# tanmayrainanda/ishara

Hardware: AMD Instinct MI355X
Metric: landmark-frames/sec training (B=256,T=384,d=256) (higher is better)
Workload: dtype bf16; 1 GPU; configs[1]: get_model(dim=256, 2 squeeze + 2 conformer blocks, kernel_sizes=[11,5,3]) CTC train step (fwd+CTC+bwd+RAdam/Lookahead, dropout on); batch_per_gpu=256, global_batch=256, frames=384, features=224, params=7577784, parallelism=dp1, ranks_seen=1

## Files before the change

### include/ishara_hip.h

```cpp
#ifndef ISHARA_HIP_H
#define ISHARA_HIP_H
#include <stdint.h>
#ifdef __cplusplus
extern "C" {
#endif

typedef struct ishara_model ishara_model;
typedef void* ishara_stream;

enum { ISHARA_F32 = 0, ISHARA_BF16 = 1, ISHARA_F16 = 2 };
enum { ISHARA_FAMILY_KERAS_HYBRID = 0, ISHARA_FAMILY_TORCH_CONFORMER = 1, ISHARA_FAMILY_TORCH_SQUEEZEFORMER = 2 };

typedef struct ishara_config {
    int32_t dim;
    int32_t num_conv_squeeze_blocks;
    int32_t num_conv_conform_blocks;
    int32_t num_kernel_sizes;
    int32_t kernel_sizes[8];
    int32_t num_conv_per_block;
    float   dropout_rate;
    int32_t num_heads;
    int32_t expansion_factor;
    int32_t transformer_kernel_size;
    int32_t frames;
// ... 69 lines not shown
                         int32_t* dist, int32_t* tlen, ishara_stream s);

int64_t ishara_ctc_beam_workspace_bytes(int32_t B, int32_t T, int32_t C, int32_t beam_width);
int ishara_ctc_beam_decode(const float* logits, int32_t B, int32_t T, int32_t C, int32_t blank, int32_t beam_width, int32_t nbest,
                           const float* lm, float alpha, float beta, void* workspace,
                           int32_t* out_idx, int32_t* out_len, float* out_score, ishara_stream s);

int64_t ishara_ctc_align_workspace_bytes(int32_t B, int32_t T, int32_t L);
int ishara_ctc_align(const float* logits, const int64_t* labels, int32_t B, int32_t T, int32_t C, int32_t L, int32_t blank,
                     void* ws, int32_t* frame_pos, int32_t* start, int32_t* end, float* conf, float* score, ishara_stream s);

typedef struct ishara_clip_aug {
    int64_t offset;
    int32_t n;
    int32_t L1;
    int32_t shift;
    int32_t L2;
    int32_t mirror;
    int32_t t0[3];
    int32_t t1[3];
    int32_t fingers[3];
} ishara_clip_aug;
enum { ISHARA_LAYOUT_FLAT = 0, ISHARA_LAYOUT_HANDS_LIPS_XY = 1 };
int ishara_clip_batch(const float* raw, const ishara_clip_aug* clips, int32_t B, int32_t T, int32_t layout,
                      float* x, ishara_stream s);
int64_t ishara_ctc_workspace_bytes(int32_t B, int32_t T, int32_t L);
int ishara_ctc_loss(const float* logits, const int64_t* labels, int32_t B, int32_t T, int32_t C,
                    int32_t L, int32_t blank, float* nll, float* dlogits, float grad_scale,
                    void* ws, ishara_stream s);
int ishara_dropout_mask(uint32_t seed, uint32_t site, int32_t rows, int32_t cols, float rate,
                        float* out, ishara_stream s);

int ishara_debug_set_as_flags(int32_t flags);
int ishara_debug_set_nt_big(int32_t on);
int ishara_debug_force_regstage(int32_t on);
int32_t ishara_debug_module_count(ishara_model* m);
int ishara_debug_module_info(ishara_model* m, int32_t i, const char** name, int32_t* in_cols, int32_t* out_cols, int32_t* first_site, int32_t* n_sites);
int ishara_debug_module_forward(ishara_model* m, int32_t i, const float* x, int32_t B, float* y, int32_t training, uint32_t seed, ishara_stream s);
int ishara_debug_module_backward(ishara_model* m, int32_t i, const float* dy, int32_t B, float* dx, ishara_stream s);
int ishara_debug_head_loss_backward(ishara_model* m, const float* logits, const int64_t* labels, int32_t B, float* loss, float* nll,
                                    float loss_scale, float* dx, ishara_stream s);

int64_t ishara_op_scratch_bytes(int32_t M, int32_t K, int32_t N);
int ishara_op_dense_fwd(int32_t dt, const void* x, const float* W, const float* bias, void* y,
                        int32_t M, int32_t K, int32_t N, int32_t act, void* scratch, ishara_stream s);
int ishara_op_dense_fwd_ex(int32_t dt, const void* x, const float* W, const float* bias, const void* resid, void* y,
                           int32_t M, int32_t K, int32_t N, int32_t act, void* scratch, ishara_stream s);
int ishara_op_dense_bwd(int32_t dt, const void* x, const float* W, const void* dy, void* dx,
                        float* dW, float* db, int32_t M, int32_t K, int32_t N, void* scratch, ishara_stream s);
int64_t ishara_op_qkv_scratch_bytes(int32_t B, int32_t T, int32_t H, int32_t dh);
int ishara_op_qkv_fwd(int32_t dt, const void* x, const float* gamma, const float* beta, float eps, const float* W, const float* bias,
                      void* q, void* k, void* vt, int32_t B, int32_t T, int32_t H, int32_t dh, int32_t head_major, void* scratch, ishara_stream s);
int ishara_op_classifier_fwd(int32_t dt, const void* x, const float* W, const float* bias, float* logits, int32_t M, int32_t K, int32_t C,
                             int32_t route, void* scratch, ishara_stream s);
int ishara_op_ctc_loss(const float* logits, const int64_t* labels, int32_t B, int32_t T, int32_t C, int32_t L, int32_t blank,
                       float* nll, float* dlogits, float grad_scale, void* ws, void* dlb, ishara_stream s);
int ishara_op_log_softmax_fwd(const float* x, float* y, int32_t M, int32_t C, int32_t ld, ishara_stream s);
int ishara_op_log_softmax_bwd(const float* dy, const float* y, float* dx, int32_t M, int32_t C, int32_t ld, ishara_stream s);
int ishara_op_layernorm_fwd(int32_t dt, const void* x, const float* gamma, const float* beta, float eps,
                            void* y, float* mean, float* rstd, int32_t M, int32_t C, ishara_stream s);
int ishara_op_layernorm_bwd(int32_t dt, const void* dy, const void* x, const float* mean, const float* rstd,
                            const float* gamma, void* dx, float* dgamma, float* dbeta, int32_t M, int32_t C,
                            ishara_stream s);
int ishara_op_dwconv_fwd(int32_t dt, int32_t inop, const void* x, const float* w, const float* bias, void* y,
                         float* ssum, float* ssq, int32_t B, int32_t T, int32_t C, int32_t k, int32_t padl,
                         ishara_stream s);
// ... 44 lines not shown
```

### ishara_amd/_lib.py

```python
from __future__ import annotations

import ctypes as C
import os

_HERE = os.path.dirname(os.path.abspath(__file__))
LIB_PATH = os.path.join(_HERE, "libishara_hip.so")

F32, BF16, F16 = 0, 1, 2
FAMILY_KERAS_HYBRID, FAMILY_TORCH_CONFORMER, FAMILY_TORCH_SQUEEZEFORMER = 0, 1, 2


class IsharaError(RuntimeError):
    pass


class Config(C.Structure):
    _fields_ = [
        ("dim", C.c_int32), ("num_conv_squeeze_blocks", C.c_int32), ("num_conv_conform_blocks", C.c_int32),
        ("num_kernel_sizes", C.c_int32), ("kernel_sizes", C.c_int32 * 8), ("num_conv_per_block", C.c_int32),
        ("dropout_rate", C.c_float), ("num_heads", C.c_int32), ("expansion_factor", C.c_int32),
        ("transformer_kernel_size", C.c_int32), ("frames", C.c_int32), ("features", C.c_int32),
        ("num_classes", C.c_int32), ("top_dim", C.c_int32), ("squeeze_expansion", C.c_int32),
        ("conformer_expansion", C.c_int32), ("head_dropout", C.c_float), ("conformer_attn_dropout", C.c_float),
        ("dtype", C.c_int32), ("max_batch", C.c_int32), ("max_label_len", C.c_int32), ("attn_impl", C.c_int32),
# ... 31 lines not shown
    "ishara_grad_bucket": (C.c_int, [_P, _I32, C.POINTER(C.c_int64), C.POINTER(C.c_int64)]),
    "ishara_grad_buckets_enable": (C.c_int, [_P]),
    "ishara_grad_bucket_wait": (C.c_int, [_P, _I32, _P]),
    "ishara_bind": (C.c_int, [_P, _P, _P, _P, _P, _P, _P, _I64]),
    "ishara_sync_weights": (C.c_int, [_P, _P]),
    "ishara_forward": (C.c_int, [_P, _P, _I32, _P, _I32, _U32, _P]),
    "ishara_encoder_forward": (C.c_int, [_P, _P, _I32, _P, _I32, _U32, _P]),
    "ishara_encoder_backward": (C.c_int, [_P, _P, _I32, _P, _P]),
    "ishara_encoder_output_frames": (_I32, [_P]),
    "ishara_loss_backward": (C.c_int, [_P, _P, _P, _I32, _P, _P, _F, _P]),
    "ishara_optimizer_step": (C.c_int, [_P, _F, _F, _P]),
    "ishara_optimizer_iterations": (_I32, [_P]),
    "ishara_optimizer_set_iterations": (C.c_int, [_P, _I32]),
    "ishara_grad_stats_workspace_bytes": (_I64, [_I64]),
    "ishara_gradient_stats": (C.c_int, [_P, _P, _I64, _F, _F, _P, _P, _P]),
    "ishara_gradient_accumulate": (C.c_int, [_P, _P, _P, _I64, _I32, _P]),
    "ishara_optimizer_step_ex": (C.c_int, [_P, _F, _F, _P, _P, _I32, _P]),
    "ishara_profile_enable": (C.c_int, [_P, _I32]),
    "ishara_profile_report": (C.c_int, [_P, C.c_char_p, _I32]),
    "ishara_greedy_decode": (C.c_int, [_P, _I32, _I32, _I32, _I32, _P, _P, _P]),
    "ishara_preprocess": (C.c_int, [_P, _P, _I32, _P, _P, _P, _I32, _P]),
    "ishara_preprocess_batch": (C.c_int, [_P, _I64, _P, _I32, _I32, _P, _P, _P, _I32, _P]),
    "ishara_edit_distance": (C.c_int, [_P, _P, _I32, _I32, _P, _I32, _P, _P, _P]),
    "ishara_ctc_beam_workspace_bytes": (_I64, [_I32, _I32, _I32, _I32]),
    "ishara_ctc_beam_decode": (C.c_int, [_P, _I32, _I32, _I32, _I32, _I32, _I32, _P, _F, _F, _P, _P, _P, _P, _P]),
    "ishara_ctc_align_workspace_bytes": (_I64, [_I32, _I32, _I32]),
    "ishara_ctc_align": (C.c_int, [_P, _P, _I32, _I32, _I32, _I32, _I32, _P, _P, _P, _P, _P, _P, _P]),
    "ishara_clip_batch": (C.c_int, [_P, _P, _I32, _I32, _I32, _P, _P]),
    "ishara_ctc_workspace_bytes": (_I64, [_I32, _I32, _I32]),
    "ishara_ctc_loss": (C.c_int, [_P, _P, _I32, _I32, _I32, _I32, _I32, _P, _P, _F, _P, _P]),
    "ishara_op_ctc_loss": (C.c_int, [_P, _P, _I32, _I32, _I32, _I32, _I32, _P, _P, _F, _P, _P, _P]),
    "ishara_dropout_mask": (C.c_int, [_U32, _U32, _I32, _I32, _F, _P, _P]),
    "ishara_debug_set_as_flags": (C.c_int, [_I32]),
    "ishara_debug_set_nt_big": (C.c_int, [_I32]),
    "ishara_debug_force_regstage": (C.c_int, [_I32]),
    "ishara_debug_module_count": (_I32, [_P]),
    "ishara_debug_module_info": (C.c_int, [_P, _I32, C.POINTER(C.c_char_p), C.POINTER(_I32), C.POINTER(_I32), C.POINTER(_I32), C.POINTER(_I32)]),
    "ishara_debug_module_forward": (C.c_int, [_P, _I32, _P, _I32, _P, _I32, _U32, _P]),
    "ishara_debug_module_backward": (C.c_int, [_P, _I32, _P, _I32, _P, _P]),
    "ishara_debug_head_loss_backward": (C.c_int, [_P, _P, _P, _I32, _P, _P, _F, _P, _P]),
    "ishara_op_scratch_bytes": (_I64, [_I32, _I32, _I32]),
    "ishara_op_dense_fwd": (C.c_int, [_I32, _P, _P, _P, _P, _I32, _I32, _I32, _I32, _P, _P]),
    "ishara_op_dense_fwd_ex": (C.c_int, [_I32, _P, _P, _P, _P, _P, _I32, _I32, _I32, _I32, _P, _P]),
    "ishara_op_dense_bwd": (C.c_int, [_I32, _P, _P, _P, _P, _P, _P, _I32, _I32, _I32, _P, _P]),
    "ishara_op_qkv_scratch_bytes": (_I64, [_I32, _I32, _I32, _I32]),
    "ishara_op_qkv_fwd": (C.c_int, [_I32, _P, _P, _P, _F, _P, _P, _P, _P, _P, _I32, _I32, _I32, _I32, _I32, _P, _P]),
    "ishara_op_classifier_fwd": (C.c_int, [_I32, _P, _P, _P, _P, _I32, _I32, _I32, _I32, _P, _P]),
    "ishara_op_log_softmax_fwd": (C.c_int, [_P, _P, _I32, _I32, _I32, _P]),
    "ishara_op_log_softmax_bwd": (C.c_int, [_P, _P, _P, _I32, _I32, _I32, _P]),
    "ishara_op_layernorm_fwd": (C.c_int, [_I32, _P, _P, _P, _F, _P, _P, _P, _I32, _I32, _P]),
    "ishara_op_layernorm_bwd": (C.c_int, [_I32, _P, _P, _P, _P, _P, _P, _P, _P, _I32, _I32, _P]),
    "ishara_op_dwconv_fwd": (C.c_int, [_I32, _I32, _P, _P, _P, _P, _P, _P, _I32, _I32, _I32, _I32, _I32, _P]),
    "ishara_op_dwconv_scratch_bytes": (_I64, [_I32, _I32]),
    "ishara_op_dwconv_fwd_scratch_bytes": (_I64, [_I32, _I32, _I32]),
    "ishara_op_dwconv_fwd_ex": (C.c_int, [_I32, _I32, _P, _P, _P, _P, _P, _P, _P, _I32, _I32, _I32, _I32, _I32, _P]),
    "ishara_op_dwconv_bwd": (C.c_int, [_I32, _I32, _P, _P, _P, _P, _P, _P, _P, _I32, _I32, _I32, _I32, _I32, _P]),
    "ishara_op_attn_scratch_bytes": (_I64, [_I32, _I32, _I32, _I32]),
    "ishara_op_attn_scratch_layout_bytes": (C.c_int, [_I32, _I32, _I32, _I32, C.POINTER(_I64)]),
    "ishara_op_attn_fwd": (C.c_int, [_I32, _P, _P, _I32, _I32, _I32, _I32, _F, _U32, _U32, _F, _I32, _P, _P]),
    "ishara_op_attn_bwd": (C.c_int, [_I32, _P, _P, _P, _I32, _I32, _I32, _I32, _F, _U32, _U32, _F, _I32, _P, _P]),
    "ishara_op_relattn_scratch_bytes": (_I64, [_I32, _I32, _I32, _I32]),
    "ishara_op_relattn_fwd": (C.c_int, [_I32] + [_P] * 9 + [_I32, _I32, _I32, _I32, _U32, _U32, _F, _P, _P]),
    "ishara_op_relattn_bwd": (C.c_int, [_I32] + [_P] * 14 + [_I32, _I32, _I32, _I32, _U32, _U32, _F, _P, _P]),
    "ishara_op_r4_subsample_scratch_bytes": (_I64, [_I32, _I32, _I32, _I32]),
    "ishara_op_r4_subsample_fwd": (C.c_int, [_I32] + [_P] * 6 + [_I32, _I32, _I32, _I32, _P, _P]),
    "ishara_op_r4_subsample_bwd": (C.c_int, [_I32] + [_P] * 10 + [_I32, _I32, _I32, _I32, _P, _P]),
# ... 45 lines not shown
```

### ishara_amd/csrc/api_ops.hip

```cpp
#include "model_types.h"

__global__ void dropout_mask_kernel(float* out, int rows, int cols, DropSpec d) {
    const size_t n = (size_t)rows * cols;
    for (size_t i = (size_t)blockIdx.x * blockDim.x + threadIdx.x; i < n; i += (size_t)gridDim.x * blockDim.x) {
        const uint32_t r = (uint32_t)(i / cols), c = (uint32_t)(i % cols);
        out[i] = (d.thr == 0u || rng_keep(rng_row_key(d.key, r), c, d.thr)) ? d.scale : 0.f;
    }
}
template <typename T>
__global__ void qkv_split_kernel(const T* qkv, T* q, T* k, T* vt, int B, int H, int Tn, int dh) {
    const int d = H * dh;
    const size_t n = (size_t)B * Tn * 3 * d;
    for (size_t i = (size_t)blockIdx.x * blockDim.x + threadIdx.x; i < n; i += (size_t)gridDim.x * blockDim.x) {
        const size_t m = i / (3 * d);
        const int col = (int)(i - m * 3 * d);
        const int h = col / (3 * dh), w = col - h * 3 * dh, part = w / dh, e = w - part * dh;
        const int b = (int)(m / Tn), t = (int)(m - (size_t)b * Tn);
        const T v = qkv[i];
        if (part == 0) q[((size_t)(b * H + h) * Tn + t) * dh + e] = v;
        else if (part == 1) k[((size_t)(b * H + h) * Tn + t) * dh + e] = v;
        else vt[((size_t)(b * H + h) * dh + e) * Tn + t] = v;
    }
}

// ... 126 lines not shown
        const size_t es = dt_size(dt);
        ldt = (int)rup(K, bk); ldn = (int)rup(N, bk);
        wt = 0;
        wn = rup(rup(N, 128) * (size_t)ldt * es, 256);
        slab = wn + rup(rup(K, 128) * (size_t)ldn * es, 256);
        total = slab + gemm_tn_slab_floats(M, K, N, dt) * sizeof(float);
    }
    int build(int dt, const float* Wm, int K, int N, char* sc, hipStream_t s) const {
        HIP_CHECK_RET(hipMemsetAsync(sc, 0, slab, s));
        return launch_make_shadow(dt, Wm, K, N, sc + wt, ldt, sc + wn, ldn, s);
    }
};
extern "C" int64_t ishara_op_scratch_bytes(int32_t M, int32_t K, int32_t N) {
    return (int64_t)OpShadow(DT_F32, K, N, M).total;
}
extern "C" int ishara_op_dense_fwd(int32_t dt, const void* x, const float* Wm, const float* bias, void* y, int32_t M, int32_t K, int32_t N, int32_t act, void* scratch, ishara_stream st) {
    OP_DT("ishara_op_dense_fwd", dt, true);
    hipStream_t s = (hipStream_t)st;
    const OpShadow sh(dt, K, N, M);
    char* sc = (char*)scratch;
    CK(sh.build(dt, Wm, K, N, sc, s));
    OpArgs no; EpiArgs ea; ea.bias = bias; ea.act = act; ea.dbg = g_dbg_epi;
    return launch_gemm_nt(dt, dt, dt, OP_NONE, x, sc + sh.wt, y, M, N, K, sh.ldt, no, ea, s);
}
extern "C" int ishara_op_dense_fwd_ex(int32_t dt, const void* x, const float* Wm, const float* bias, const void* resid, void* y,
                                      int32_t M, int32_t K, int32_t N, int32_t act, void* scratch, ishara_stream st) {
    OP_DT("ishara_op_dense_fwd_ex", dt, true);
    hipStream_t s = (hipStream_t)st;
    const OpShadow sh(dt, K, N, M);
    char* sc = (char*)scratch;
    CK(sh.build(dt, Wm, K, N, sc, s));
    OpArgs no; EpiArgs ea; ea.bias = bias; ea.act = act; ea.resid = resid; ea.dbg = g_dbg_epi;
    return launch_gemm_nt(dt, dt, dt, OP_NONE, x, sc + sh.wt, y, M, N, K, sh.ldt, no, ea, s);
}
extern "C" int ishara_op_dense_bwd(int32_t dt, const void* x, const float* Wm, const void* dy, void* dx, float* dW, float* db,
                                   int32_t M, int32_t K, int32_t N, void* scratch, ishara_stream st) {
    OP_DT("ishara_op_dense_bwd", dt, false);
    hipStream_t s = (hipStream_t)st;
    const OpShadow sh(dt, K, N, M);
    char* sc = (char*)scratch;
    CK(sh.build(dt, Wm, K, N, sc, s));
    OpArgs no; EpiArgs ea;
    if (dx) CK(launch_gemm_nt(dt, dt, dt, OP_NONE, dy, sc + sh.wn, dx, M, K, N, sh.ldn, no, ea, s));
    return launch_gemm_tn(dt, dt, dt, OP_NONE, OP_NONE, x, dy, dW, db, (float*)(sc + sh.slab), M, K, N, no, no, s);
}
static void qkv_scratch_layout(int B, int T, int H, int dh, size_t& xn, size_t& mean, size_t& rstd, size_t& total) {
    const int M = B * T, d = H * dh;
    xn = rup(OpShadow(DT_F32, d, 3 * d, M).total, 256);
    mean = xn + rup((size_t)M * d * 4, 256);
    rstd = mean + rup((size_t)M * 4, 256);
    total = rstd + rup((size_t)M * 4, 256);
}
extern "C" int64_t ishara_op_qkv_scratch_bytes(int32_t B, int32_t T, int32_t H, int32_t dh) {
    if (B < 1 || T < 1 || H < 1 || dh < 1) return -1;
    size_t xn, mean, rstd, total;
    qkv_scratch_layout(B, T, H, dh, xn, mean, rstd, total);
    return (int64_t)total;
}
extern "C" int ishara_op_qkv_fwd(int32_t dt, const void* x, const float* gamma, const float* beta, float eps, const float* Wm, const float* bias,
                                 void* q, void* k, void* vt, int32_t B, int32_t T, int32_t H, int32_t dh, int32_t head_major, void* scratch, ishara_stream st) {
    OP_DT("ishara_op_qkv_fwd", dt, true);
    if (B < 1 || T < 1 || H < 1 || dh < 1 || T % 8 != 0 || dh % 8 != 0 || (head_major != 0 && head_major != 1)) {
        ishara_set_error("ishara_op_qkv_fwd: B=%d T=%d H=%d dh=%d head_major=%d unsupported (T, dh multiples of 8; head_major 0 / 1)", B, T, H, dh, head_major); return -1;
    }
    const int d = H * dh, M = B * T;
    if ((gamma != nullptr) != (beta != nullptr) || (gamma && d > 512)) { ishara_set_error("ishara_op_qkv_fwd: LayerNorm needs both gamma and beta and H*dh <= 512 (H*dh=%d)", d); return -1; }
// ... 318 lines not shown
```

### ishara_amd/csrc/gemm_nt.hip

```cpp
#include "gemm_tile.h"

template <typename TA, typename TM, typename TC, int OP>
__global__ __launch_bounds__(256) void gemm_nt_kernel(const TA* __restrict__ A, const TM* __restrict__ Bt, TC* __restrict__ C,
                                                      int M, int N, int K, int ldb, int a_vec_ok, OpArgs oa, EpiArgs ea) {
    __shared__ __attribute__((aligned(16))) char smem[65536];
    constexpr int BK = MmaCfg<TM>::BK;
    const int tid = threadIdx.x, lane = tid & 63, wid = tid >> 6, wr = wid >> 1, wc = wid & 1;
    const int nMt = (M + 127) >> 7, nNt = (N + 127) >> 7;
    int mt, nt;
    {
        const int id = blockIdx.x;
        if ((nMt & 7) == 0) { const int xcd = id & 7, local = id >> 3; mt = (local / nNt) * 8 + xcd; nt = local % nNt; }
        else { mt = id / nNt; nt = id % nNt; }
    }
    const int m0 = mt << 7, n0 = nt << 7;
    const int nk = (K + BK - 1) / BK;

    u32x4 ra[4], rb[4];
    f32x4 acc[4][4];
#pragma unroll
    for (int i = 0; i < 4; ++i)
#pragma unroll
        for (int j = 0; j < 4; ++j) acc[i][j] = f32x4{0.f, 0.f, 0.f, 0.f};

// ... 473 lines not shown
static int run_nt(const void* A, const void* Bt, void* C, int M, int N, int K, int ldb, const OpArgs& oa, const EpiArgs& ea, hipStream_t s) {
    const int nMt = (M + 127) / 128, nNt = (N + 127) / 128;
    const int a_vec_ok = (((size_t)K * sizeof(TA)) % 16 == 0) && (((uintptr_t)A) % 16 == 0);
    hipLaunchKernelGGL((gemm_nt_kernel<TA, TM, TC, OP>), dim3(nMt * nNt), dim3(256), 0, s,
                       (const TA*)A, (const TM*)Bt, (TC*)C, M, N, K, ldb, a_vec_ok, oa, ea);
    return launch_rc();
}

template <typename TA, typename TM, typename TC>
static int run_nt_op(int op, const void* A, const void* Bt, void* C, int M, int N, int K, int ldb, const OpArgs& oa, const EpiArgs& ea, hipStream_t s) {
    switch (op) {
        case OP_NONE: return run_nt<TA, TM, TC, OP_NONE>(A, Bt, C, M, N, K, ldb, oa, ea, s);
        case OP_SWISH: return run_nt<TA, TM, TC, OP_SWISH>(A, Bt, C, M, N, K, ldb, oa, ea, s);
        case OP_COLAFFINE: return run_nt<TA, TM, TC, OP_COLAFFINE>(A, Bt, C, M, N, K, ldb, oa, ea, s);
        case OP_DROPMASK: return run_nt<TA, TM, TC, OP_DROPMASK>(A, Bt, C, M, N, K, ldb, oa, ea, s);
        default: ishara_set_error("gemm_nt: unsupported operand op %d", op); return -1;
    }
}

int g_force_regstage = 0;

NtRoute gemm_nt_route(int dtA, int dtM, int dtC, int op, const void* A, int M, int N, int K, int ldb, const EpiArgs& ea) {
    const bool pro = ea.ln_gamma || ea.pa_P;
    if (dtM == DT_F16) {
        if (op != OP_NONE) return NT_REFUSED;
        if (dtA == DT_F16 && g_force_regstage == 0 && (K == 256 || K == 512) && ldb % 64 == 0 && ((uintptr_t)A) % 16 == 0 && gemm_nt_as_applicable(dtC, M, N, K, ldb, ea)) return NT_AS_F16;
        if (pro) return NT_REFUSED;
        return (dtA == DT_F16 && (dtC == DT_F16 || dtC == DT_F32)) || (dtA == DT_F32 && dtC == DT_F16) ? NT_REG : NT_REFUSED;
    }
    if (pro && (op != OP_NONE || !gemm_nt_as_prologue_ok(dtA, dtM, dtC, M, N, K, ldb, ea))) return NT_REFUSED;
    if (g_force_regstage == 0 && gemm_nt_big_applicable(dtA, dtM, dtC, op, A, M, N, K, ldb, ea)) return NT_BIG;
    const int bk = dtM == DT_BF16 ? 32 : 16;
    const bool dma_ok = op == OP_NONE && dtA == dtM && K % bk == 0 && ldb % (2 * bk) == 0 && ((uintptr_t)A) % 16 == 0;
    if (dma_ok && g_force_regstage == 0 && dtM == DT_BF16 && gemm_nt_as_applicable(dtC, M, N, K, ldb, ea)) return NT_AS;
    const bool dma_dt = (dtM == DT_F32 && dtC == DT_F32) || (dtM == DT_BF16 && (dtC == DT_BF16 || dtC == DT_F32));
    if (dma_ok && dma_dt && (g_force_regstage == 0 || g_force_regstage == 3) && N % 4 == 0 && (ea.mode != EPI_QKV || ea.dh % 4 == 0)) return NT_TILE_T;
    if (dma_ok && dma_dt && g_force_regstage != 1) return NT_GLDS;
    if (dtA == dtM && dtM == dtC && (dtM == DT_F32 || dtM == DT_BF16)) return NT_REG;
    if (dtM == DT_BF16 && op == OP_NONE && ((dtA == DT_F32 && dtC == DT_BF16) || (dtA == DT_BF16 && dtC == DT_F32))) return NT_REG;
    return NT_REFUSED;
}

int launch_gemm_nt(int dtA, int dtM, int dtC, int op, const void* A, const void* Bt, void* C,
                   int M, int N, int K, int ldb, const OpArgs& oa, const EpiArgs& ea, hipStream_t s) {
    if (M <= 0 || N <= 0 || K <= 0) { ishara_set_error("gemm_nt: bad shape %d %d %d", M, N, K); return -1; }
    if ((dt_is16(dtA) && K % 8 != 0) || (dtA == DT_F32 && K % 4 != 0) || ((uintptr_t)A) % 16 != 0) {
        ishara_set_error("gemm_nt: A rows must be 16-byte aligned (K=%d)", K); return -1;
    }
    if (ea.mode == EPI_QKV && (ea.T % 8 != 0 || N % 8 != 0 || ea.dh % 8 != 0)) {
        ishara_set_error("gemm_nt: QKV split needs T, dh multiples of 8 (T=%d dh=%d)", ea.T, ea.dh); return -1;
    }
    const bool f16m = dtM == DT_F16;
    int rc = 1;
    switch (gemm_nt_route(dtA, dtM, dtC, op, A, M, N, K, ldb, ea)) {
        case NT_REFUSED:
            if (f16m && op != OP_NONE) ishara_set_error("gemm_nt: f16 operands take no operand transform");
            else if (f16m && (ea.ln_gamma || ea.pa_P)) ishara_set_error("gemm_nt: f16 operand prologue on a shape the A-stationary kernel does not take");
            else if (f16m) ishara_set_error("gemm_nt: unsupported f16 dtype combination %d/%d/%d", dtA, dtM, dtC);
            else if (ea.ln_gamma || ea.pa_P) ishara_set_error("gemm_nt: operand prologue requested for a shape the A-stationary kernel does not take (check gemm_nt_as_prologue_ok first)");
            else ishara_set_error("gemm_nt: unsupported dtype combination %d/%d/%d op %d", dtA, dtM, dtC, op);
            return -1;
        case NT_AS_F16: rc = launch_gemm_nt_as_f16(dtC, A, Bt, C, M, N, K, ldb, ea, s); break;
        case NT_BIG: rc = launch_gemm_nt_big(dtA, dtM, dtC, op, A, Bt, C, M, N, K, ldb, ea, s); break;
        case NT_AS: rc = launch_gemm_nt_as(dtC, A, Bt, C, M, N, K, ldb, ea, s); break;
        case NT_TILE_T:
            if (dtM == DT_F32) return run_nt_t<float, float>(A, Bt, C, M, N, K, ldb, ea, s);
            return dtC == DT_BF16 ? run_nt_t<bf16, bf16>(A, Bt, C, M, N, K, ldb, ea, s) : run_nt_t<bf16, float>(A, Bt, C, M, N, K, ldb, ea, s);
        case NT_GLDS:
            if (dtM == DT_F32) return run_nt_glds<float, float>(A, Bt, C, M, N, K, ldb, ea, s);
            return dtC == DT_BF16 ? run_nt_glds<bf16, bf16>(A, Bt, C, M, N, K, ldb, ea, s) : run_nt_glds<bf16, float>(A, Bt, C, M, N, K, ldb, ea, s);
        case NT_REG:
            if (f16m && dtA == DT_F32) return run_nt<float, f16, f16, OP_NONE>(A, Bt, C, M, N, K, ldb, oa, ea, s);
            if (f16m) return dtC == DT_F16 ? run_nt<f16, f16, f16, OP_NONE>(A, Bt, C, M, N, K, ldb, oa, ea, s) : run_nt<f16, f16, float, OP_NONE>(A, Bt, C, M, N, K, ldb, oa, ea, s);
            if (dtA != dtM) return run_nt<float, bf16, bf16, OP_NONE>(A, Bt, C, M, N, K, ldb, oa, ea, s);
            if (dtC != dtM) return run_nt<bf16, bf16, float, OP_NONE>(A, Bt, C, M, N, K, ldb, oa, ea, s);
            return dtM == DT_F32 ? run_nt_op<float, float, float>(op, A, Bt, C, M, N, K, ldb, oa, ea, s) : run_nt_op<bf16, bf16, bf16>(op, A, Bt, C, M, N, K, ldb, oa, ea, s);
    }
    if (rc == 1) { ishara_set_error("gemm_nt: internal error: the kernel gemm_nt_route chose refused the call (M=%d N=%d K=%d)", M, N, K); return -1; }
    return rc;
}

const char* gemm_nt_kernel_name(int dtA, int dtM, int dtC, int op, const void* A, int M, int N, int K, int ldb, const EpiArgs& ea) {
    const NtRoute route = gemm_nt_route(dtA, dtM, dtC, op, A, M, N, K, ldb, ea);
    if (dtM == DT_F16) return "gemm_nt_kernel<f16>";
    switch (route) {
        case NT_BIG: return "gemm_nt_big_kernel<bf16>";
        case NT_AS: return gemm_nt_as_name(dtC, K, ea, M, N);
        case NT_TILE_T: return dtM == DT_F32 ? "gemm_nt_t_kernel<f32,f32>" : (dtC == DT_F32 ? "gemm_nt_t_kernel<bf16,f32>" : "gemm_nt_t_kernel<bf16,bf16>");
        case NT_GLDS: return dtM == DT_F32 ? "gemm_nt_glds_kernel<f32,f32>" : (dtC == DT_F32 ? "gemm_nt_glds_kernel<bf16,f32>" : "gemm_nt_glds_kernel<bf16,bf16>");
        default: break;
    }
    if (dtA == DT_F32 && dtM == DT_BF16) return "gemm_nt_kernel<f32,bf16,bf16>";
    if (dtM == DT_F32) return "gemm_nt_kernel<f32,f32,f32>";
    return dtC == DT_F32 ? "gemm_nt_kernel<bf16,bf16,f32>" : "gemm_nt_kernel<bf16,bf16,bf16>";
}
```

### ishara_amd/csrc/kernels.h

```cpp
#pragma once
#include "common.h"
#include "../../include/ishara_hip.h"

enum DType : int { DT_F32 = 0, DT_BF16 = 1, DT_F16 = 2 };
static inline size_t dt_size(int dt) { return dt == DT_F32 ? 4 : 2; }
static inline bool dt_is16(int dt) { return dt != DT_F32; }

enum : int { OP_NONE = 0, OP_SWISH = 1, OP_COLAFFINE = 2, OP_ROWSCALE = 3, OP_DROPMASK = 4 };
struct OpArgs {
    const float* c1 = nullptr;
    const float* c0 = nullptr;
    const float* rs = nullptr;
    int T = 1;
    DropSpec drop = {0, 0, 1.f};
};

enum : int { ACT_NONE = 0, ACT_SWISH = 1, ACT_RELU = 2 };
enum : int { DACT_NONE = 0, DACT_SWISH = 1, DACT_POS = 2 };
enum : int { EPI_STD = 0, EPI_QKV = 1 };
struct EpiArgs {
    const float* bias = nullptr;
    const float* addtab = nullptr;
    int tab_period = 1;
    void* pre_out = nullptr;
    int act = ACT_NONE;
    DropSpec drop = {0, 0, 1.f};
    const float* rowscale = nullptr;
    int T = 1;
    int rowscale_bias = 0;
    int dact = DACT_NONE;
    const void* aux = nullptr;
    const void* resid = nullptr;
    int mode = EPI_STD;
    void* q = nullptr; void* k = nullptr; void* vt = nullptr;
    int H = 1, dh = 1;
    int dbg = 0;
    const float* ln_gamma = nullptr;
    const float* ln_beta = nullptr;
    float ln_eps = 0.f;
    float* ln_mean = nullptr;
    float* ln_rstd = nullptr;
    const float* pa_P = nullptr;
    const float* pa_Q = nullptr;
    void* pro_out = nullptr;
    int head_major = 1;
    int ldc = 0, n_valid = 0;
    int as_flags = -1;
};

int launch_gemm_nt(int dtA, int dtM, int dtC, int op, const void* A, const void* Bt, void* C,
                   int M, int N, int K, int ldb, const OpArgs& oa, const EpiArgs& ea, hipStream_t s);
enum NtRoute { NT_REFUSED, NT_AS_F16, NT_BIG, NT_AS, NT_TILE_T, NT_GLDS, NT_REG };
NtRoute gemm_nt_route(int dtA, int dtM, int dtC, int op, const void* A, int M, int N, int K, int ldb, const EpiArgs& ea);
const char* gemm_nt_kernel_name(int dtA, int dtM, int dtC, int op, const void* A, int M, int N, int K, int ldb, const EpiArgs& ea);
bool gemm_nt_as_applicable(int dtC, int M, int N, int K, int ldb, const EpiArgs& ea);
bool gemm_nt_as_prologue_ok(int dtA, int dtM, int dtC, int M, int N, int K, int ldb, const EpiArgs& ea);
const char* gemm_nt_as_name(int dtC, int K, const EpiArgs& ea, int M, int N);
int launch_gemm_nt_as(int dtC, const void* A, const void* Bt, void* C, int M, int N, int K, int ldb, const EpiArgs& ea, hipStream_t s);
int launch_gemm_nt_as_f16(int dtC, const void* A, const void* Bt, void* C, int M, int N, int K, int ldb, const EpiArgs& ea, hipStream_t s);
bool gemm_nt_big_applicable(int dtA, int dtM, int dtC, int op, const void* A, int M, int N, int K, int ldb, const EpiArgs& ea);
int launch_gemm_nt_big(int dtA, int dtM, int dtC, int op, const void* A, const void* Bt, void* C, int M, int N, int K, int ldb, const EpiArgs& ea, hipStream_t s);

size_t gemm_tn_slab_floats(int M, int Ka, int Nb, int dtM);
#define RED_MAXJOBS 48
struct RedJob { const float* slab; float* out0; float* out1; size_t stride; int n0, n, splits, nb, nbv, first_block; };
struct RedSink { RedJob job[RED_MAXJOBS]; int njobs = 0; int nblocks = 0; };
extern RedSink* g_red_sink;
void launch_reduce_slabs(const float* slab, float* out, int n, int splits, size_t stride, hipStream_t s);
void launch_reduce_slabs2(const float* slab, float* out0, int n0, float* out1, int n1, int splits, size_t stride, hipStream_t s, int nb = 0, int nbv = 0);
bool reduce_cols_ok(const float* slab, const float* out0, const float* out1, int n0, int n, size_t stride);
bool reduce_sink_full();
int launch_reduce_flush(RedSink* sink, hipStream_t s);
bool gemm_tn_bias_rowscale_ok(int dtA, int dtB, int dtM, int M, int Ka, int Nb, int T);
struct TnDefer { float* slab[2] = {nullptr, nullptr}; int turn = 0; bool pending = false;
                 const float* p_slab = nullptr; float* p_out0 = nullptr; float* p_out1 = nullptr; int p_n0 = 0, p_n = 0, p_splits = 0; size_t p_stride = 0; int p_nb = 0, p_nbv = 0; };
int launch_gemm_tn_flush(TnDefer* defer, hipStream_t s);
struct TnPsa { const float* P = nullptr; const float* Q = nullptr;
               const void* W = nullptr; int ldw = 0;
               float* G = nullptr; float* Rpart = nullptr; int T = 0;
               int dbg = 0; };
bool gemm_tn_psa_ok(int dtA, int dtB, int dtM, int M, int Ka, int Nb, int T);
int launch_gemm_tn(int dtA, int dtB, int dtM, int opA, int opB, const void* A, const void* B,
                   float* out, float* dbias, float* slab, int M, int Ka, int Nb,
                   const OpArgs& oa, const OpArgs& ob, hipStream_t s, int ka_valid = 0, int nb_valid = 0,
                   const float* bias_rowscale = nullptr, int bias_T = 0, TnDefer* defer = nullptr, const TnPsa* psa = nullptr);
int launch_dense_narrow(int dt, const void* A, const void* Wt, int ldt, const float* bias, float* C, int M, int N, int K, hipStream_t s);
int launch_pack_rows_bf16(const float* x, void* xb, int M, int F, int Kp, hipStream_t s, int dt = DT_BF16);

enum TnRoute { TN_REFUSED, TN_BIG, TN_TR, TN_TR_BRS, TN_TR_PSA, TN_REG };
TnRoute gemm_tn_route(int dtA, int dtB, int dtM, int opA, int opB, int M, int Ka, int Nb, int ka_valid, int nb_valid, bool brs, int brsT, bool psa, int psaT);
const char* gemm_tn_kernel_name(int dtA, int dtB, int dtM, int opA, int opB, int M, int Ka, int Nb, int ka_valid = 0, int nb_valid = 0,
                                const float* bias_rowscale = nullptr, int bias_T = 0, const TnPsa* psa = nullptr);
// ... 115 lines not shown
```

Baseline: 6.741 million frames/s.

## Add specialized K=512,N=256 bf16 GEMM with LDS ring pipeline and fused epilogue

Adds a dedicated bf16 GEMM kernel for the K=512, N=256 dense shape. It streams weights through a 4-stage LDS ring using global_load_lds and double-buffers A rows in registers. Each block processes 384 rows in two passes, and the next pass's prefetch overlaps the epilogue. The epilogue fuses residual, dropout, rowscale and an optional per-column affine prologue. The router prefers this path over the existing AS kernel for large M. Hand-tuned vmcnt waits and inline asm make correctness depend on exact instruction counts.

```diff
diff --git a/include/ishara_hip.h b/include/ishara_hip.h
--- a/include/ishara_hip.h
+++ b/include/ishara_hip.h
@@ -125,6 +125,7 @@
                         float* out, ishara_stream s);
 
 int ishara_debug_set_as_flags(int32_t flags);
+const char* ishara_debug_dense_kernel_name(int32_t dt, int32_t M, int32_t K, int32_t N, int32_t act, int32_t with_resid);
 int ishara_debug_set_nt_big(int32_t on);
 int ishara_debug_force_regstage(int32_t on);
 int32_t ishara_debug_module_count(ishara_model* m);
diff --git a/ishara_amd/_lib.py b/ishara_amd/_lib.py
--- a/ishara_amd/_lib.py
+++ b/ishara_amd/_lib.py
@@ -87,6 +87,7 @@
     "ishara_op_ctc_loss": (C.c_int, [_P, _P, _I32, _I32, _I32, _I32, _I32, _P, _P, _F, _P, _P, _P]),
     "ishara_dropout_mask": (C.c_int, [_U32, _U32, _I32, _I32, _F, _P, _P]),
     "ishara_debug_set_as_flags": (C.c_int, [_I32]),
+    "ishara_debug_dense_kernel_name": (C.c_char_p, [_I32, _I32, _I32, _I32, _I32, _I32]),
     "ishara_debug_set_nt_big": (C.c_int, [_I32]),
     "ishara_debug_force_regstage": (C.c_int, [_I32]),
     "ishara_debug_module_count": (_I32, [_P]),
diff --git a/ishara_amd/csrc/api_ops.hip b/ishara_amd/csrc/api_ops.hip
--- a/ishara_amd/csrc/api_ops.hip
+++ b/ishara_amd/csrc/api_ops.hip
@@ -182,6 +182,13 @@
     CK(sh.build(dt, Wm, K, N, sc, s));
     OpArgs no; EpiArgs ea; ea.bias = bias; ea.act = act; ea.resid = resid; ea.dbg = g_dbg_epi;
     return launch_gemm_nt(dt, dt, dt, OP_NONE, x, sc + sh.wt, y, M, N, K, sh.ldt, no, ea, s);
+}
+extern "C" const char* ishara_debug_dense_kernel_name(int32_t dt, int32_t M, int32_t K, int32_t N, int32_t act, int32_t with_resid) {
+    if (!op_dt_ok("ishara_debug_dense_kernel_name", dt, true) || M < 1 || K < 1 || N < 1) return "";
+    const OpShadow sh(dt, K, N, M);
+    const void* aligned = reinterpret_cast<const void*>(uintptr_t(256));
+    EpiArgs ea; ea.bias = reinterpret_cast<const float*>(aligned); ea.act = act; ea.resid = with_resid ? aligned : nullptr; ea.dbg = g_dbg_epi;
+    return gemm_nt_kernel_name(dt, dt, dt, OP_NONE, aligned, M, N, K, sh.ldt, ea);
 }
 extern "C" int ishara_op_dense_bwd(int32_t dt, const void* x, const float* Wm, const void* dy, void* dx, float* dW, float* db,
                                    int32_t M, int32_t K, int32_t N, void* scratch, ishara_stream st) {
diff --git a/ishara_amd/csrc/gemm_cs.hip b/ishara_amd/csrc/gemm_cs.hip
--- /dev/null
+++ b/ishara_amd/csrc/gemm_cs.hip
@@ -0,0 +1,315 @@
+#include <cstdio>
+#include <cstdlib>
+#include <map>
+#include "common.h"
+#include "kernels.h"
+
+enum { CS_RESID = 1, CS_DROP = 8, CS_ROWSCALE = 16 };
+#define CS_K 512
+#define CS_N 256
+#define CS_ROWS 384
+#define CS_NST 8
+#define CS_RING 4
+#define CS_STAGE 32768
+#define CS_DPW 4
+#define CS_LDS (CS_RING * CS_STAGE + CS_N * 4 + 2 * CS_K * 4)
+#define CS_DEFAULT_FLAGS 115
+#define CS_MIN_M 49153
+
+typedef __attribute__((ext_vector_type(4))) uint32_t cs_u32x4;
+
+template <int N> DEVI void cs_wait_vm() { static_assert(N >= 0 && N < 64, "vmcnt is 6 bits"); asm volatile("s_waitcnt vmcnt(%0)" ::"n"(N) : "memory"); }
+template <int N0, int NP> DEVI void cs_wait(bool counted, bool pout) {
+    if (!counted) cs_wait_vm<0>(); else if (pout) cs_wait_vm<NP>(); else cs_wait_vm<N0>();
+}
+template <int OFF> DEVI cs_u32x4 cs_ld16(const void* p) {
+    cs_u32x4 r;
+    asm volatile("global_load_dwordx4 %0, %1, off offset:%2" : "=v"(r) : "v"(p), "n"(OFF) : "memory");
+    return r;
+}
+DEVI void cs_pin(cs_u32x4& r) { asm volatile("" : "+v"(r)); }
+DEVI void cs_mfma(bool first, f32x4& acc, const bf16x8& b, const cs_u32x4& a) {
+    if (first) asm volatile("v_mfma_f32_16x16x32_bf16 %0, %1, %2, 0" : "=&v"(acc) : "v"(b), "v"(a));
+    else asm volatile("v_mfma_f32_16x16x32_bf16 %0, %1, %2, %0" : "+v"(acc) : "v"(b), "v"(a));
+}
+DEVI int cs_swz(int r) { return (r & 2) | (((r >> 4) & 1) << 2); }
+DEVI void cs_unpack(const cs_u32x4& r, float (&v)[8]) {
+#pragma unroll
+    for (int h = 0; h < 4; ++h) { v[2 * h] = __uint_as_float(r[h] << 16); v[2 * h + 1] = __uint_as_float(r[h] & 0xffff0000u); }
+}
+DEVI void cs_st_pk(bf16* p, const bf16x8& t, bool nt) {
+    if (nt) __builtin_nontemporal_store(t, reinterpret_cast<bf16x8*>(p)); else *reinterpret_cast<bf16x8*>(p) = t;
+}
+
+struct CsLane {
+    const bf16* bsrc[CS_DPW];
+    int off0, off1;
+    int wid, c, g;
+};
+template <int RT> struct CsRows {
+    const bf16* ap[RT];
+    int mrow[RT];
+    cs_u32x4 a[3][RT][2];
+};
+template <int RT> DEVI void cs_rows_init(CsRows<RT>& r, const bf16* __restrict__ A, int M, int mw, const CsLane& L) {
+#pragma unroll
+    for (int i = 0; i < RT; ++i) {
+        r.mrow[i] = min(mw + 16 * i + L.c, M - 1);
+        r.ap[i] = A + (size_t)r.mrow[i] * CS_K + L.g * 8;
+    }
+}
+template <int RT, int S> DEVI void cs_load_a(CsRows<RT>& r) {
+#pragma unroll
+    for (int i = 0; i < RT; ++i) {
+        r.a[S % 3][i][0] = cs_ld16<S * 128>(r.ap[i]);
+        r.a[S % 3][i][1] = cs_ld16<S * 128 + 64>(r.ap[i]);
+    }
+}
+template <int S> DEVI void cs_issue_w(const CsLane& L, char* smem) {
+#pragma unroll
+    for (int t = 0; t < CS_DPW; ++t) {
+        const bf16* src = L.bsrc[t];
+        asm volatile("" : "+v"(src));
+        __builtin_amdgcn_global_load_lds((const __attribute__((address_space(1))) void*)(src + S * 64),
+                                         (__attribute__((address_space(3))) void*)(smem + (S % CS_RING) * CS_STAGE + (L.wid * CS_DPW + t) * 1024), 16, 0, 0);
+    }
+}
+template <int RT> DEVI void cs_prefetch(CsRows<RT>& r, const CsLane& L, char* smem) {
+    cs_load_a<RT, 0>(r);
+    cs_load_a<RT, 1>(r);
+    cs_issue_w<0>(L, smem);
+    cs_issue_w<1>(L, smem);
+    cs_issue_w<2>(L, smem);
+}
+#define CS_PREFETCH_OPS(RT) (2 * 2 * (RT) + 3 * CS_DPW)
+
+template <int MASK, int PRO, int RT, int E, int S>
+DEVI void cs_stage(CsRows<RT>& r, const CsLane& L, char* smem, const float* pq_s, f32x4 (&acc)[8][2][RT], bf16* pro_out, int M, int mw,
+                   bool full, bool pout, bool nt_side) {
+    constexpr int NA = 2 * RT, D = CS_DPW;
+    if constexpr (S == 0) cs_wait<2 * D + E, 2 * D + E>(full, pout);
+    else if constexpr (S == 1) cs_wait<2 * D + E + NA, 2 * D + E + NA + NA>(full, pout);
+    else if constexpr (S <= 5) cs_wait<2 * D + NA, 2 * D + NA + 2 * NA>(full, pout);
+    else if constexpr (S == 6) cs_wait<D + NA, D + NA + 2 * NA>(full, pout);
+    else cs_wait<0, 2 * NA>(full, pout);
+    asm volatile("s_waitcnt lgkmcnt(0)" ::: "memory");
+    __builtin_amdgcn_s_barrier();
+    if constexpr (S + 2 < CS_NST) cs_load_a<RT, S + 2>(r);
+    if constexpr (S + 3 < CS_NST) cs_issue_w<S + 3>(L, smem);
+    constexpr int B = S % 3;
+#pragma unroll
+    for (int i = 0; i < RT; ++i) { cs_pin(r.a[B][i][0]); cs_pin(r.a[B][i][1]); }
+    if constexpr (PRO == 2) {
+#pragma unroll
+        for (int kt = 0; kt < 2; ++kt) {
+            const float* cp = pq_s + 64 * S + 32 * kt + 8 * L.g;
+            const f32x4 w0 = *reinterpret_cast<const f32x4*>(cp), w1 = *reinterpret_cast<const f32x4*>(cp + 4);
+            const f32x4 b0 = *reinterpret_cast<const f32x4*>(cp + CS_K), b1 = *reinterpret_cast<const f32x4*>(cp + CS_K + 4);
+            float wv[8], bv[8];
+#pragma unroll
+            for (int e = 0; e < 4; ++e) { wv[e] = w0[e]; wv[4 + e] = w1[e]; bv[e] = b0[e]; bv[4 + e] = b1[e]; }
+#pragma unroll
+            for (int i = 0; i < RT; ++i) {
+                float v[8];
+                cs_unpack(r.a[B][i][kt], v);
+                bf16x8 t;
+#pragma unroll
+                for (int e = 0; e < 8; ++e) t[e] = (bf16)(v[e] * wv[e] + bv[e]);
+                r.a[B][i][kt] = __builtin_bit_cast(cs_u32x4, t);
+                if (pout && (full || mw + 16 * i + L.c < M))
+                    cs_st_pk(pro_out + (size_t)r.mrow[i] * CS_K + L.g * 8 + 64 * S + 32 * kt, t, nt_side);
+            }
+        }
+    }
+    const char* st = smem + (S % CS_RING) * CS_STAGE;
+    auto frag = [&](int q, int jj) { return *reinterpret_cast<const bf16x8*>(st + ((q >> 3) ? L.off1 : L.off0) + (32 * (q & 7) + 4 * jj) * 128); };
+    bf16x8 b0 = frag(0, 0), b1 = frag(0, 1), c0 = frag(1, 0), c1 = frag(1, 1);
+    if constexpr (PRO != 0) asm volatile("s_nop 1");
+#pragma unroll
+    for (int q = 0; q < 16; ++q) {
+        const int kt = q >> 3, p = q & 7;
+        bf16x8 n0 = c0, n1 = c1;
+        if (q + 2 < 16) { n0 = frag(q + 2, 0); n1 = frag(q + 2, 1); }
+        asm volatile("" ::: "memory");
+#pragma unroll
+        for (int i = 0; i < RT; ++i) {
+            cs_mfma(S == 0 && q < 8, acc[p][0][i], b0, r.a[B][i][kt]);
+            cs_mfma(S == 0 && q < 8, acc[p][1][i], b1, r.a[B][i][kt]);
+        }
+        b0 = c0; b1 = c1; c0 = n0; c1 = n1;
+    }
+}
+
+template <int MASK, int PRO, int RT, int E, typename HAND>
+DEVI void cs_pass(CsRows<RT>& r, const CsLane& L, bf16* __restrict__ C, int M, const EpiArgs& ea, char* smem, const float* bias_s, const float* pq_s,
+                  int m_base, float rsc, int hops, HAND hand) {
+    const int mw = m_base + L.wid * 16 * RT;
+    const bool full = m_base + 128 * RT <= M;
+    const bool pout = PRO != 0 && ea.pro_out != nullptr;
+    const bool nt_side = (ea.as_flags & 2) != 0;
+    constexpr bool f_resid = (MASK & CS_RESID) != 0, f_drop = (MASK & CS_DROP) != 0, f_rowscale = (MASK & CS_ROWSCALE) != 0;
+    f32x4 acc[8][2][RT];
+    bf16* po = reinterpret_cast<bf16*>(ea.pro_out);
+    cs_stage<MASK, PRO, RT, E, 0>(r, L, smem, pq_s, acc, po, M, mw, full, pout, nt_side);
+    cs_stage<MASK, PRO, RT, E, 1>(r, L, smem, pq_s, acc, po, M, mw, full, pout, nt_side);
+    cs_stage<MASK, PRO, RT, E, 2>(r, L, smem, pq_s, acc, po, M, mw, full, pout, nt_side);
+    cs_stage<MASK, PRO, RT, E, 3>(r, L, smem, pq_s, acc, po, M, mw, full, pout, nt_side);
+    cs_stage<MASK, PRO, RT, E, 4>(r, L, smem, pq_s, acc, po, M, mw, full, pout, nt_side);
+    cs_stage<MASK, PRO, RT, E, 5>(r, L, smem, pq_s, acc, po, M, mw, full, pout, nt_side);
+    cs_stage<MASK, PRO, RT, E, 6>(r, L, smem, pq_s, acc, po, M, mw, full, pout, nt_side);
+    cs_stage<MASK, PRO, RT, E, 7>(r, L, smem, pq_s, acc, po, M, mw, full, pout, nt_side);
+
+    asm volatile("s_nop 15");
+    size_t eoff[RT];
+#pragma unroll
+    for (int i = 0; i < RT; ++i) eoff[i] = (size_t)r.mrow[i] * CS_N + 8 * L.g;
+    cs_u32x4 rs[RT][8];
+    if constexpr (f_resid) {
+        const bf16* resid = reinterpret_cast<const bf16*>(ea.resid);
+#pragma unroll
+        for (int i = 0; i < RT; ++i) {
+            const bf16* rp = resid + eoff[i];
+            rs[i][0] = cs_ld16<0>(rp);   rs[i][1] = cs_ld16<64>(rp);  rs[i][2] = cs_ld16<128>(rp); rs[i][3] = cs_ld16<192>(rp);
+            rs[i][4] = cs_ld16<256>(rp); rs[i][5] = cs_ld16<320>(rp); rs[i][6] = cs_ld16<384>(rp); rs[i][7] = cs_ld16<448>(rp);
+        }
+    }
+    asm volatile("s_waitcnt lgkmcnt(0)" ::: "memory");
+    __builtin_amdgcn_s_barrier();
+    hand();
+    if constexpr (f_resid) {
+        if (hops) cs_wait_vm<CS_PREFETCH_OPS(1)>(); else cs_wait_vm<0>();
+#pragma unroll
+        for (int i = 0; i < RT; ++i)
+#pragma unroll
+            for (int p = 0; p < 8; ++p) cs_pin(rs[i][p]);
+    }
+    uint32_t rk[RT];
+#pragma unroll
+    for (int i = 0; i < RT; ++i) rk[i] = f_drop ? rng_row_key(ea.drop.key, (uint32_t)(mw + 16 * i + L.c)) : 0u;
+#pragma unroll
+    for (int i = 0; i < RT; ++i) {
+        const int m = mw + 16 * i + L.c;
+        if (!full && m >= M) continue;
+#pragma unroll
+        for (int p = 0; p < 8; ++p) {
+            const int n = 32 * p + 8 * L.g;
+            float bias[8];
+#pragma unroll
+            for (int h = 0; h < 2; ++h) {
+                const f32x4 bv = *reinterpret_cast<const f32x4*>(bias_s + n + 4 * h);
+#pragma unroll
+                for (int e = 0; e < 4; ++e) bias[4 * h + e] = bv[e];
+            }
+            float v[8];
+            const float bsc = (f_rowscale && ea.rowscale_bias) ? rsc : 1.f;
+#pragma unroll
+            for (int e = 0; e < 4; ++e) { v[e] = acc[p][0][i][e] + bias[e] * bsc; v[4 + e] = acc[p][1][i][e] + bias[4 + e] * bsc; }
+            if constexpr (f_drop) rng_apply<8>(rk[i], (uint32_t)n, ea.drop.thr, ea.drop.scale, v);
+            if (f_rowscale && !ea.rowscale_bias) {
+#pragma unroll
+                for (int e = 0; e < 8; ++e) v[e] *= rsc;
+            }
+            if constexpr (f_resid) {
+                float x[8];
+                cs_unpack(rs[i][p], x);
+#pragma unroll
+                for (int e = 0; e < 8; ++e) v[e] += x[e];
+            }
+            store8(C + eoff[i] + 32 * p, v);
+        }
+    }
+}
+
+template <int MASK, int PRO>
+__global__ __launch_bounds__(512, 1) void gemm_nt_cs_kernel(const bf16* __restrict__ A, const bf16* __restrict__ Bt, bf16* __restrict__ C, int M, int ldb, EpiArgs ea) {
+    extern __shared__ __attribute__((aligned(16))) char cs_smem[];
+    float* bias_s = reinterpret_cast<float*>(cs_smem + CS_RING * CS_STAGE);
+    float* pq_s = bias_s + CS_N;
+    const int tid = threadIdx.x, lane = tid & 63;
+    const int m_base = blockIdx.x * CS_ROWS;
+    const int bsm = min(m_base, M - 1) / max(ea.T, 1);
+    for (int n = tid; n < CS_N; n += 512) bias_s[n] = ea.bias ? ea.bias[n] : 0.f;
+    if constexpr (PRO == 2) {
+        const float* c0 = ea.pa_P + (size_t)bsm * CS_K;
+        const float* c1 = ea.pa_Q + (size_t)bsm * CS_K;
+        for (int x = tid; x < CS_K; x += 512) { pq_s[x] = c0[x]; pq_s[CS_K + x] = c1[x]; }
+    }
+    float rsc = 1.f;
+    if constexpr ((MASK & CS_ROWSCALE) != 0) rsc = ea.rowscale[bsm];
+    __syncthreads();
+    asm volatile("" : "+v"(rsc));
+
+    CsLane L;
+    L.wid = __builtin_amdgcn_readfirstlane(tid >> 6);
+    L.c = lane & 15; L.g = lane >> 4;
+#pragma unroll
+    for (int t = 0; t < CS_DPW; ++t) {
+        const int rr = (L.wid * CS_DPW + t) * 8 + (lane >> 3), p = lane & 7;
+        L.bsrc[t] = Bt + (size_t)rr * ldb + ((p ^ cs_swz(rr)) << 3);
+    }
+    const int frow = 8 * (L.c >> 2) + (L.c & 3);
+    const int sx = L.g ^ cs_swz(frow);
+    L.off0 = frow * 128 + (sx << 4);
+    L.off1 = frow * 128 + ((sx ^ 4) << 4);
+
+    const bool two = m_base + 256 < M;
+    CsRows<2> r1;
+    CsRows<1> r2;
+    cs_rows_init<2>(r1, A, M, m_base + L.wid * 32, L);
+    cs_prefetch<2>(r1, L, cs_smem);
+    cs_pass<MASK, PRO, 2, 0>(r1, L, C, M, ea, cs_smem, bias_s, pq_s, m_base, rsc, two ? CS_PREFETCH_OPS(1) : 0, [&]() {
+        if (two) {
+            cs_rows_init<1>(r2, A, M, m_base + 256 + L.wid * 16, L);
+            cs_prefetch<1>(r2, L, cs_smem);
+        }
+    });
+    if (two) cs_pass<MASK, PRO, 1, 16>(r2, L, C, M, ea, cs_smem, bias_s, pq_s, m_base + 256, rsc, 0, []() {});
+}
+
+static int cs_mask_of(const EpiArgs& ea) {
+    return (ea.resid ? 1 : 0) | (ea.dact != DACT_NONE ? 2 : 0) | (ea.act != ACT_NONE ? 4 : 0) | (ea.drop.thr ? 8 : 0) | (ea.rowscale ? 16 : 0) |
+           (ea.pre_out ? 32 : 0) | (ea.mode == EPI_QKV ? 64 : 0) | (ea.addtab ? 128 : 0);
+}
+static int cs_flags(const EpiArgs& ea) {
+    static const int v = getenv("ISHARA_AS_FLAGS") ? atoi(getenv("ISHARA_AS_FLAGS")) : CS_DEFAULT_FLAGS;
+    return ea.as_flags >= 0 ? ea.as_flags : (g_as_flags_override >= 0 ? g_as_flags_override : v);
+}
+bool gemm_nt_cs_applicable(int dtC, int M, int N, int K, int ldb, const EpiArgs& ea) {
+    if (dtC != DT_BF16 || K != CS_K || N != CS_N || M < 1 || ldb < CS_K || ldb % 8 != 0) return false;
+    const int flags = cs_flags(ea);
+    if (!(flags & 64)) return false;
+    if (ea.n_valid || ea.dbg || (ea.ldc && ea.ldc != CS_N) || ea.ln_gamma) return false;
+    if (!(flags & 128) && M < CS_MIN_M) return false;
+    const int mask = cs_mask_of(ea);
+    if (ea.pa_P) return ea.pa_Q && ea.T > 0 && ea.T % CS_ROWS == 0 && (mask == CS_RESID || mask == (CS_RESID | CS_ROWSCALE));
+    return mask == 0 || mask == CS_RESID || mask == (CS_RESID | CS_DROP);
+}
+const char* gemm_nt_cs_name(const EpiArgs& ea) {
+    static std::map<int, std::string> names;
+    const int mask = cs_mask_of(ea), pro = ea.pa_P ? 2 : 0;
+    auto it = names.find(mask | pro << 8);
+    if (it == names.end()) {
+        char buf[64];
+        snprintf(buf, sizeof buf, "gemm_nt_cs_kernel<%d,%d>", mask, pro);
+        it = names.emplace(mask | pro << 8, buf).first;
+    }
+    return it->second.c_str();
+}
+template <int MASK, int PRO>
+static int cs_launch(const void* A, const void* Bt, void* C, int M, int ldb, const EpiArgs& ea, hipStream_t s) {
+    static int ready = 0;
+    if (!ready) ready = hipFuncSetAttribute(reinterpret_cast<const void*>(gemm_nt_cs_kernel<MASK, PRO>), hipFuncAttributeMaxDynamicSharedMemorySize, CS_LDS) == hipSuccess ? 1 : -1;
+    if (ready < 0) { ishara_set_error("gemm_nt_cs: %d bytes of LDS refused", CS_LDS); return -1; }
+    hipLaunchKernelGGL((gemm_nt_cs_kernel<MASK, PRO>), dim3((M + CS_ROWS - 1) / CS_ROWS), dim3(512), CS_LDS, s, (const bf16*)A, (const bf16*)Bt, (bf16*)C, M, ldb, ea);
+    return launch_rc();
+}
+int launch_gemm_nt_cs(int dtC, const void* A, const void* Bt, void* C, int M, int N, int K, int ldb, const EpiArgs& ea_in, hipStream_t s) {
+    if (!gemm_nt_cs_applicable(dtC, M, N, K, ldb, ea_in)) return 1;
+    EpiArgs ea = ea_in;
+    ea.as_flags = cs_flags(ea_in);
+    const int mask = cs_mask_of(ea);
+    if (ea.pa_P) return mask == CS_RESID ? cs_launch<CS_RESID, 2>(A, Bt, C, M, ldb, ea, s) : cs_launch<CS_RESID | CS_ROWSCALE, 2>(A, Bt, C, M, ldb, ea, s);
+    if (mask == 0) return cs_launch<0, 0>(A, Bt, C, M, ldb, ea, s);
+    if (mask == CS_RESID) return cs_launch<CS_RESID, 0>(A, Bt, C, M, ldb, ea, s);
+    return cs_launch<CS_RESID | CS_DROP, 0>(A, Bt, C, M, ldb, ea, s);
+}
diff --git a/ishara_amd/csrc/gemm_nt.hip b/ishara_amd/csrc/gemm_nt.hip
--- a/ishara_amd/csrc/gemm_nt.hip
+++ b/ishara_amd/csrc/gemm_nt.hip
@@ -529,6 +529,7 @@
     if (g_force_regstage == 0 && gemm_nt_big_applicable(dtA, dtM, dtC, op, A, M, N, K, ldb, ea)) return NT_BIG;
     const int bk = dtM == DT_BF16 ? 32 : 16;
     const bool dma_ok = op == OP_NONE && dtA == dtM && K % bk == 0 && ldb % (2 * bk) == 0 && ((uintptr_t)A) % 16 == 0;
+    if (dma_ok && g_force_regstage == 0 && dtM == DT_BF16 && gemm_nt_cs_applicable(dtC, M, N, K, ldb, ea)) return NT_CS;
     if (dma_ok && g_force_regstage == 0 && dtM == DT_BF16 && gemm_nt_as_applicable(dtC, M, N, K, ldb, ea)) return NT_AS;
     const bool dma_dt = (dtM == DT_F32 && dtC == DT_F32) || (dtM == DT_BF16 && (dtC == DT_BF16 || dtC == DT_F32));
     if (dma_ok && dma_dt && (g_force_regstage == 0 || g_force_regstage == 3) && N % 4 == 0 && (ea.mode != EPI_QKV || ea.dh % 4 == 0)) return NT_TILE_T;
@@ -559,6 +560,7 @@
             return -1;
         case NT_AS_F16: rc = launch_gemm_nt_as_f16(dtC, A, Bt, C, M, N, K, ldb, ea, s); break;
         case NT_BIG: rc = launch_gemm_nt_big(dtA, dtM, dtC, op, A, Bt, C, M, N, K, ldb, ea, s); break;
+        case NT_CS: rc = launch_gemm_nt_cs(dtC, A, Bt, C, M, N, K, ldb, ea, s); break;
         case NT_AS: rc = launch_gemm_nt_as(dtC, A, Bt, C, M, N, K, ldb, ea, s); break;
         case NT_TILE_T:
             if (dtM == DT_F32) return run_nt_t<float, float>(A, Bt, C, M, N, K, ldb, ea, s);
@@ -582,6 +584,7 @@
     if (dtM == DT_F16) return "gemm_nt_kernel<f16>";
     switch (route) {
         case NT_BIG: return "gemm_nt_big_kernel<bf16>";
+        case NT_CS: return gemm_nt_cs_name(ea);
         case NT_AS: return gemm_nt_as_name(dtC, K, ea, M, N);
         case NT_TILE_T: return dtM == DT_F32 ? "gemm_nt_t_kernel<f32,f32>" : (dtC == DT_F32 ? "gemm_nt_t_kernel<bf16,f32>" : "gemm_nt_t_kernel<bf16,bf16>");
         case NT_GLDS: return dtM == DT_F32 ? "gemm_nt_glds_kernel<f32,f32>" : (dtC == DT_F32 ? "gemm_nt_glds_kernel<bf16,f32>" : "gemm_nt_glds_kernel<bf16,bf16>");
diff --git a/ishara_amd/csrc/kernels.h b/ishara_amd/csrc/kernels.h
--- a/ishara_amd/csrc/kernels.h
+++ b/ishara_amd/csrc/kernels.h
@@ -50,7 +50,7 @@
 
 int launch_gemm_nt(int dtA, int dtM, int dtC, int op, const void* A, const void* Bt, void* C,
                    int M, int N, int K, int ldb, const OpArgs& oa, const EpiArgs& ea, hipStream_t s);
-enum NtRoute { NT_REFUSED, NT_AS_F16, NT_BIG, NT_AS, NT_TILE_T, NT_GLDS, NT_REG };
+enum NtRoute { NT_REFUSED, NT_AS_F16, NT_BIG, NT_CS, NT_AS, NT_TILE_T, NT_GLDS, NT_REG };
 NtRoute gemm_nt_route(int dtA, int dtM, int dtC, int op, const void* A, int M, int N, int K, int ldb, const EpiArgs& ea);
 const char* gemm_nt_kernel_name(int dtA, int dtM, int dtC, int op, const void* A, int M, int N, int K, int ldb, const EpiArgs& ea);
 bool gemm_nt_as_applicable(int dtC, int M, int N, int K, int ldb, const EpiArgs& ea);
@@ -58,6 +58,9 @@
 const char* gemm_nt_as_name(int dtC, int K, const EpiArgs& ea, int M, int N);
 int launch_gemm_nt_as(int dtC, const void* A, const void* Bt, void* C, int M, int N, int K, int ldb, const EpiArgs& ea, hipStream_t s);
 int launch_gemm_nt_as_f16(int dtC, const void* A, const void* Bt, void* C, int M, int N, int K, int ldb, const EpiArgs& ea, hipStream_t s);
+bool gemm_nt_cs_applicable(int dtC, int M, int N, int K, int ldb, const EpiArgs& ea);
+const char* gemm_nt_cs_name(const EpiArgs& ea);
+int launch_gemm_nt_cs(int dtC, const void* A, const void* Bt, void* C, int M, int N, int K, int ldb, const EpiArgs& ea, hipStream_t s);
 bool gemm_nt_big_applicable(int dtA, int dtM, int dtC, int op, const void* A, int M, int N, int K, int ldb, const EpiArgs& ea);
 int launch_gemm_nt_big(int dtA, int dtM, int dtC, int op, const void* A, const void* Bt, void* C, int M, int N, int K, int ldb, const EpiArgs& ea, hipStream_t s);
 
```

Result: faster. 6.904 million frames/s, median of 6 (+2.4%).
